# EmilyJrxx/YOLO_PPF_Pose_Estimation

Measured on AMD Instinct MI355X. Metric: PPF pair-matches/sec (accumulator votes) per cropped scene, higher is better.
Workload: dtype u32 votes / f64 pair features

## Files before the change

yolo_ppf_pose_estimation_amd/csrc/ppf_match_host.h:

```cpp
#ifndef PPF_MATCH_HOST_H
#define PPF_MATCH_HOST_H

extern "C" {

ppf_status ppf_workspace_create(ppf_workspace** out) {
  if (!out) return fail(PPF_ERR_INVALID, "ppf_workspace_create: NULL");
  *out = new (std::nothrow) ppf_workspace();
  if (!*out) return fail(PPF_ERR_NOMEM, "ppf_workspace_create: out of memory");
  return PPF_OK;
}
ppf_status ppf_workspace_destroy(ppf_workspace* ws) {
  if (!ws) return PPF_OK;
  delete ws;
  return PPF_OK;
}
ppf_status ppf_workspace_set_option(ppf_workspace* ws, int option, double value) {
  if (!ws) return fail(PPF_ERR_INVALID, "ppf_workspace_set_option: NULL");
  switch (option) {
    case PPF_OPT_HIT_FRACTION:
      if (!(value > 0 && value <= 1)) return fail(PPF_ERR_INVALID, "ppf_workspace_set_option: hit fraction must be in (0, 1]");
      ws->hit_frac = value;
      ws->frac_known = true;
      return PPF_OK;
    case PPF_OPT_GROUP_ROUND_BUCKETS:
      if (!(value >= 0 && value <= 1e9)) return fail(PPF_ERR_INVALID, "ppf_workspace_set_option: bad bucket count");
      ws->round_buckets_cap = (int)value;
      return PPF_OK;
    case PPF_OPT_CLUSTER_SERIAL:
      ws->cluster_serial = value != 0;
      return PPF_OK;
    case PPF_OPT_ACC32:
      if (!(value == 0 || value == 1 || value == 2 || value == 3)) return fail(PPF_ERR_INVALID, "ppf_workspace_set_option: PPF_OPT_ACC32 takes 0 .. 3");
      ws->force_acc32 = value == 1;
      ws->acc32_policy = value == 1 ? 0 : (int)value;
      ws->heavy_votes = ~0ull;
      if (value != 0) ws->acc32 = false;
      return PPF_OK;
    case PPF_OPT_BATCH_REFS:
      if (!(value >= 0 && value <= 1e9)) return fail(PPF_ERR_INVALID, "ppf_workspace_set_option: bad batch size");
      ws->batch_refs_cap = (int)value;
      return PPF_OK;
    case PPF_OPT_RUN_STAGING:
      if (!(value >= 0 && value <= 1e9)) return fail(PPF_ERR_INVALID, "ppf_workspace_set_option: bad run staging size");
      ws->run_seg_cap = (int)value;
      return PPF_OK;
    case PPF_OPT_TABLE_FRACTION:
      if (!(value > 0 && value <= 1)) return fail(PPF_ERR_INVALID, "ppf_workspace_set_option: table fraction must be in (0, 1]");
      ws->tbl_frac = std::min(TBL_FRAC_MAX, value);
      return PPF_OK;
    default:
      return fail(PPF_ERR_INVALID, "ppf_workspace_set_option: unknown option %d", option);
  }
}
ppf_status ppf_workspace_enable_timing(ppf_workspace* ws, int on) {
  if (!ws) return fail(PPF_ERR_INVALID, "ppf_workspace_enable_timing: NULL");
  if (on && !ws->ev[0])
    for (auto& e : ws->ev) HIPCHK(hipEventCreate(&e));
  ws->timing = on != 0;
  return PPF_OK;
}

static ppf_status check_match_args(const ppf_model* m, const void* scene, int ns, int sstride, int snoff, const void* edge, int ne,
                                   int estride, int enoff, const ppf_match_params* p) {
  if (!m) return fail(PPF_ERR_NOT_TRAINED, "The model is not trained. Cannot match without training");
  if (!scene || ns <= 0 || bad_layout(sstride, snoff) || !p) return fail(PPF_ERR_INVALID, "match: bad scene argument");
  if (edge && (ne <= 0 || bad_layout(estride, enoff))) return fail(PPF_ERR_INVALID, "match: bad edge argument");
  if (!(p->relative_scene_sample_step <= 1 && p->relative_scene_sample_step > 0))
    return fail(PPF_ERR_INVALID, "match: relativeSceneSampleStep must be in (0, 1]");
  if (!p->presampled && !(p->relative_scene_distance > 0)) return fail(PPF_ERR_INVALID, "match: relativeSceneDistance must be > 0");
  if (p->ref_stride < 1 || p->ref_offset < 0) return fail(PPF_ERR_INVALID, "match: bad ref_offset/ref_stride");
  int dev = 0;
  HIPCHK(hipGetDevice(&dev));
  if (dev != m->device)
    return fail(PPF_ERR_INVALID, "match: the model lives on device %d, the calling thread's current device is %d", m->device, dev);
  return PPF_OK;
}

static ppf_status prepare_scene(ppf_workspace* ws, const float* d_scene, int ns, int sstride, int snoff, const float* d_edge, int ne,
                                int estride, int enoff, const ppf_match_params* params, hipStream_t st) {
  auto load = [&](CloudDev& dst, const float* d_src, int rows, int stride, int noff) -> ppf_status {
    if (params->presampled) return dst.load_device(d_src, rows, stride, noff, st);
    return device_sample_cloud(d_src, rows, stride, noff, (float)params->relative_scene_distance, dst, nullptr, st);
  };
  ppf_status s = load(ws->surf, d_scene, ns, sstride, snoff);
  if (s != PPF_OK) return s;
  if (d_edge) s = load(ws->edge, d_edge, ne, estride, enoff);
  ws->has_edge = d_edge != nullptr;
  return s;
}

static ppf_status match_prepared(const ppf_model* m, ppf_workspace* ws, const ppf_match_params* params, hipStream_t st, bool retry = false);

ppf_status ppf_match_device(const ppf_model* m, ppf_workspace* ws, const float* d_scene, int ns, int sstride, int snoff,
                            const float* d_edge, int ne, int estride, int enoff, const ppf_match_params* params, void* stream) {
  if (!ws) return fail(PPF_ERR_INVALID, "ppf_match_device: workspace is NULL");
  if (!m) return fail(PPF_ERR_NOT_TRAINED, "The model is not trained. Cannot match without training");
  if (!have_device()) return fail(PPF_ERR_HIP, "ppf_match_device: no HIP device (this engine has no CPU fallback)");
  ppf_status s = check_match_args(m, d_scene, ns, sstride, snoff, d_edge, ne, estride, enoff, params);
  if (s != PPF_OK) return s;
  hipStream_t st = (hipStream_t)stream;
  s = prepare_scene(ws, d_scene, ns, sstride, snoff, d_edge, ne, estride, enoff, params, st);
  if (s != PPF_OK) return s;
  return match_prepared(m, ws, params, st);
}

static ppf_workspace::Learned* workspace_learned(ppf_workspace* ws, const ppf_model* m, bool create) {
  for (auto& fm : ws->frac_by_model)
    if (fm.model_serial == m->serial) return &fm;
  if (!create) return nullptr;
  if (ws->frac_by_model.size() >= 16) ws->frac_by_model.erase(ws->frac_by_model.begin());
  ws->frac_by_model.push_back({m->serial, 0.25, 0.4, TBL_FRAC_START});
  return &ws->frac_by_model.back();
}

static void workspace_remember_frac(ppf_workspace* ws) {
  if (!ws->model || !ws->frac_known) return;
  ppf_workspace::Learned* fm = workspace_learned(ws, ws->model, true);
  fm->hit = ws->hit_frac; fm->run = ws->run_frac; fm->tbl = ws->tbl_frac;
}

static void workspace_hold_model(ppf_workspace* ws, const ppf_model* m) {
  if (ws->model == m) return;
  ppf_model* old = ws->model;
  ws->model = const_cast<ppf_model*>(m);
  if (ws->model_owns_me) return;
  if (ws->model) ws->model->refcount.fetch_add(1);
  if (old) (void)ppf_model_release(old);
}

ppf_workspace::~ppf_workspace() {
  sync_device(device);
  for (auto& e : ev)
    if (e) (void)hipEventDestroy(e);
  for (auto& e : batch_ev)
    if (e) (void)hipEventDestroy(e);
  if (model && !model_owns_me) (void)ppf_model_release(model);
  if (h_sum) (void)hipHostFree(h_sum);
}

constexpr double HIT_SCRATCH_BYTES = 8.0 + 8.0 + 2.0 + 16.0 / 6.0;

static void launch_pairs(const MatchArgs& va, bool darboux, hipStream_t st) {
  const dim3 grid(va.pair_chunks, va.n_ref), block(PAIR_BLOCK);
  const dim3 ogrid((unsigned)std::min(va.n_ref, 1024)), oblock(256);
  if (darboux) {
    if (va.same_cloud) k_pairs<true, false><<<grid, block, 0, st>>>(va);
    else k_pairs<true, true><<<grid, block, 0, st>>>(va);
    if (!va.count_only) { if (va.same_cloud) k_pairs_odd<true, false><<<ogrid, oblock, 0, st>>>(va); else k_pairs_odd<true, true><<<ogrid, oblock, 0, st>>>(va); }
  } else {
    if (va.same_cloud) k_pairs<false, false><<<grid, block, 0, st>>>(va);
    else k_pairs<false, true><<<grid, block, 0, st>>>(va);
    if (!va.count_only) { if (va.same_cloud) k_pairs_odd<false, false><<<ogrid, oblock, 0, st>>>(va); else k_pairs_odd<false, true><<<ogrid, oblock, 0, st>>>(va); }
  }
}

static ppf_status match_prepared(const ppf_model* m, ppf_workspace* ws, const ppf_match_params* params, hipStream_t st, bool retry) {
  ppf_status s = PPF_OK;
  const bool d_edge = ws->has_edge;
  if (ws->model != m) {
    workspace_remember_frac(ws);
    ws->acc32 = false;
    ws->heavy_votes = ~0ull;
    if (const ppf_workspace::Learned* fm = workspace_learned(ws, m, false)) {
      ws->hit_frac = fm->hit; ws->run_frac = fm->run; ws->tbl_frac = fm->tbl;
      ws->frac_known = true;
    } else if (!ws->frac_by_model.empty()) {
      ws->frac_known = false;
    }
  }
  workspace_hold_model(ws, m);
  HIPCHK(hipGetDevice(&ws->device));
  ws->params = *params;
  ws->stream = st;
  ws->clustered = false;
  ws->checked = false;
  ws->sum_valid = false;
  ws->final_poses.clear();
  const int retries = retry ? ws->stats.n_retries : 0;
  memset(&ws->stats, 0, sizeof(ws->stats));
  ws->stats.n_retries = retries;
  const int rows = ws->surf.n;
  const int scene_step = (int)(1.0 / params->relative_scene_sample_step);
  const int n_ref_total = (rows + scene_step - 1) / scene_step;
  const int n_ref = n_ref_total > params->ref_offset ? (n_ref_total - params->ref_offset + params->ref_stride - 1) / params->ref_stride : 0;
  ws->rows = rows;
  ws->n_ref_total = n_ref_total;
  ws->n_ref = n_ref;
  ws->n_batches = 0;
  ws->stats.n_scene_sampled = rows;
  ws->stats.n_paired = d_edge ? ws->edge.n : rows;
  ws->stats.n_ref = n_ref;
  ws->pending = true;
  if (n_ref == 0) return PPF_OK;

  const int T = m->info.n_tiles;
  HIPCHK(ws->partial.reserve((size_t)n_ref * T * 2));
  HIPCHK(ws->half_edge.reserve((size_t)n_ref * T * 2));
  HIPCHK(ws->ovf_items.reserve((size_t)n_ref * T));
  if (ws->acc32_policy == 3) {
    HIPCHK(ws->item_votes.reserve((size_t)n_ref * T));
    HIPCHK(ws->need_hist.reserve(2 * ACC_HIST));
  }
  const size_t n_cnt = (size_t)n_ref * T + n_ref + 16;
  HIPCHK(ws->counters.reserve(n_cnt));
  HIPCHK(ws->votes.reserve(n_ref));
  HIPCHK(ws->raw_poses.reserve(n_ref));
  if (ws->timing) HIPCHK(hipEventRecord(ws->ev[0], st));
  if (ws->acc_dump)
    HIPCHK(hipMemsetAsync(ws->acc_dump, 0, (size_t)n_ref * (size_t)m->info.n_ref * (size_t)m->info.num_angles * sizeof(uint32_t), st));
  if (ws->acc32_policy == 3) {
    HIPCHK(hipMemsetAsync(ws->need_hist.p, 0, 2 * ACC_HIST * sizeof(unsigned long long), st));
    HIPCHK(hipMemsetAsync(ws->item_votes.p, 0, (size_t)n_ref * T * sizeof(unsigned long long), st));
  }

  MatchArgs va;
  memset(&va, 0, sizeof(va));
  va.surf = ws->surf.view();
  va.paired = d_edge ? ws->edge.view() : ws->surf.view();
  va.same_cloud = d_edge ? 0 : 1;
  va.scene_step = scene_step; va.ref_offset = params->ref_offset; va.ref_stride = params->ref_stride;
  va.slotmap = m->slotmap.p; va.slot_mask = m->info.slots - 1;
  va.key_lut = m->key_lut.p; va.kd = m->kd;
  va.bucket_off = m->bucket_off.p; va.n_buckets = (int)m->info.n_buckets;
  va.records = m->records.p;
  va.n_tiles = T; va.tile_refs = m->info.tile_refs; va.num_angles = m->info.num_angles; va.n_model = m->info.n_ref;
  va.angle_step = m->info.angle_step; va.dist_step = m->info.distance_step;
  va.partial = ws->partial.p;
  va.edge = ws->half_edge.p;
  va.ovf_items = ws->ovf_items.p;
  va.cellsum = ws->counters.p;
  va.pairs = ws->counters.p + (size_t)n_ref * T;
  va.tally = ws->counters.p + (size_t)n_ref * T + n_ref + 2;
  va.acc_dump = ws->acc_dump;
  va.bucket_total = m->bucket_total.p;
  va.bucket_mid = m->bucket_mid.p;
  va.key_exact = m->params.key_equality == PPF_KEY_EXACT;
  const bool acc32_all = ws->force_acc32 || (ws->acc32 && ws->acc32_policy == 0);
  va.item_votes = (!acc32_all && ws->acc32_policy == 3) ? ws->item_votes.p : nullptr;
  va.heavy_votes = ws->heavy_votes;
  const bool darboux = m->params.feature == PPF_FEATURE_DARBOUX;
  va.pair_radius = params->pair_radius;
  va.agg_min_hits = (params->vote_mode == PPF_VOTE_DIRECT || params->alpha_range_2pi || m->info.num_angles > AGG_MAX_ANGLES) ? 0 : PPF_AGG_MIN_HITS;
  const int n_paired = va.paired.n;
  va.pair_chunks = (n_paired + PAIR_BLOCK * PAIRS_PER_THREAD - 1) / (PAIR_BLOCK * PAIRS_PER_THREAD);
  const uint32_t round_cap = ws->round_buckets_cap > 0 ? (uint32_t)std::min(ws->round_buckets_cap, GROUP_MAX_BUCKETS) : (uint32_t)GROUP_MAX_BUCKETS;
  va.n_rounds = std::max(1, (int)((m->info.n_buckets + round_cap - 1) / round_cap));
  va.round_buckets = (int)std::min<uint32_t>(std::max<uint32_t>(m->info.n_buckets, 1u), round_cap);

  const bool cursors_new = !ws->cursors.p;
  HIPCHK(ws->cursors.reserve(CUR_WORDS));
  va.cursors = ws->cursors.p;
  if (cursors_new) HIPCHK(hipMemsetAsync(ws->cursors.p, 0, CUR_WORDS * sizeof(uint32_t), st));
  va.n_counters = n_cnt;
  va.n_ovf_items = (unsigned long long)n_ref * T;
  if (!ws->frac_known) {
    HIPCHK(hipMemsetAsync(ws->cursors.p, 0, CUR_WORDS * sizeof(uint32_t), st));
    va.count_only = 1;
    va.stripe_bits = 6;
    for (int base = 0; base < n_ref; base += 32768) {
      va.ref_base = base;
      va.n_ref = std::min(32768, n_ref - base);
      launch_pairs(va, darboux, st);
      HIPCHK(hipGetLastError());
    }
    va.count_only = 0;
    std::vector<uint32_t> cw(CUR_SORTED);
    HIPCHK(hipMemcpyAsync(cw.data(), ws->cursors.p, cw.size() * sizeof(uint32_t), hipMemcpyDeviceToHost, st));
    HIPCHK(host_stream_sync(st));
    unsigned long long hits = 0;
    for (int sidx = 0; sidx < POOL_STRIPES; sidx++)
      hits += (unsigned long long)cw[sidx * CUR_STRIDE] | ((unsigned long long)cw[sidx * CUR_STRIDE + 1] << 32);
    const double pairs_total = (double)n_ref * (double)n_paired;
    ws->hit_frac = std::min(1.0, std::max(1e-3, 1.06 * (double)hits / std::max(1.0, pairs_total)));
    ws->frac_known = true;
  }
  const double frac = std::min(1.0, std::max(ws->hit_frac, 1e-3));
  const double hits_per_ref = std::max(64.0, frac * (double)n_paired);
  const double tbl_frac = !va.agg_min_hits ? 0.0 : frac >= 1.0 ? TBL_FRAC_MAX : std::min(TBL_FRAC_MAX, ws->tbl_frac);
  int batch = (int)std::min<double>((double)n_ref, std::max(1.0, (double)HIT_BYTES_BUDGET / (hits_per_ref * (HIT_SCRATCH_BYTES + tbl_frac * TBL_BYTES))));
  batch = (int)std::min<double>((double)batch, std::max(1.0, 2.0e9 / hits_per_ref));
  batch = std::min(batch, 32768);
  if (ws->batch_refs_cap > 0) batch = std::min(batch, ws->batch_refs_cap);
  const bool worst_case = frac >= 1.0;
  const double est = hits_per_ref * (double)batch;
  const uint32_t wg_hits = PAIR_BLOCK * PAIRS_PER_THREAD;
  int stripe_bits = 6;
  while (stripe_bits > 0 && ((size_t)batch * va.pair_chunks >> stripe_bits) < 512) stripe_bits--;
  if (worst_case) stripe_bits = 0;
  const uint32_t n_stripes = 1u << stripe_bits;
  const uint32_t stripe_cap = worst_case ? (uint32_t)std::min<double>(4.0e9 / n_stripes, (double)batch * va.pair_chunks * wg_hits)
                                         : (uint32_t)(est / n_stripes * 1.04) + 2 * wg_hits;
  const uint32_t sorted_cap = (uint32_t)std::min(4.0e9, est + 4096.0);
  const uint32_t run_cap = worst_case ? sorted_cap : (uint32_t)std::min<double>((double)sorted_cap, std::max(est * std::min(1.0, ws->run_frac), 64.0 * batch) + 1024.0);
  HIPCHK(ws->frames.reserve((size_t)batch * 12));
  HIPCHK(ws->raw.fit((size_t)stripe_cap * n_stripes));
  HIPCHK(ws->chunk_desc.reserve((size_t)batch * va.pair_chunks));
  HIPCHK(ws->hit_count.reserve(batch));
  HIPCHK(ws->s_a64.fit(sorted_cap));
  const uint32_t table_cap = !va.agg_min_hits ? 1u : (uint32_t)std::min(1.0e9, std::max(est * (worst_case ? TBL_FRAC_MAX : tbl_frac), 4.0 * batch) + 256.0);
  HIPCHK(ws->runs.fit(run_cap));
  HIPCHK(ws->tables.fit((size_t)table_cap * TBL_BYTES));
  HIPCHK(ws->table_desc.fit(table_cap));
  HIPCHK(ws->run_blocks.reserve((size_t)batch * va.n_rounds));
  HIPCHK(ws->work.reserve(batch));
  HIPCHK(ws->perm.reserve(batch));
  HIPCHK(ws->perm_group.reserve(batch));
  HIPCHK(ws->ovf_list.reserve((size_t)batch * T));
  va.ovf_list = ws->ovf_list.p;
  ws->stats.scratch_bytes = ws->frames.bytes() + ws->raw.bytes() + ws->cursors.bytes() + ws->chunk_desc.bytes() + ws->hit_count.bytes() +
                            ws->s_a64.bytes() + ws->runs.bytes() + ws->run_blocks.bytes() + ws->tables.bytes() + ws->table_desc.bytes() +
                            ws->work.bytes() + ws->perm.bytes() + ws->perm_group.bytes();
  va.frames = ws->frames.p;
  va.raw = ws->raw.p; va.stripe_cap = stripe_cap; va.stripe_bits = stripe_bits;
  va.chunk_desc = ws->chunk_desc.p; va.hit_count = ws->hit_count.p;
  va.s_a64 = ws->s_a64.p; va.sorted_cap = sorted_cap;
  va.runs = ws->runs.p; va.run_cap = run_cap; va.run_blocks = ws->run_blocks.p;
  va.tables = ws->tables.p; va.table_desc = ws->table_desc.p; va.table_cap = table_cap;
  va.work = ws->work.p; va.perm = ws->perm.p; va.perm_group = ws->perm_group.p;

  const size_t acc_words = (size_t)vote_lds_words(m->info.tile_refs, m->info.num_angles);
  va.run_seg = vote_run_seg(acc_words, (size_t)LDS_BYTES);
  if (ws->run_seg_cap > 0) va.run_seg = std::max(64, std::min(va.run_seg, ws->run_seg_cap / 64 * 64));
  const size_t lds = vote_lds_fixed(va.run_seg) + acc_words * 4;
  if (lds > (size_t)LDS_BYTES) return fail(PPF_ERR_INVALID, "match: model tile of %d reference points does not fit the LDS accumulator", m->info.tile_refs);
  const size_t group_lds = (size_t)((va.round_buckets + 1) & ~1) * sizeof(uint32_t) + (size_t)((va.pair_chunks + 2) & ~1) * sizeof(uint32_t) * 2;
  if (group_lds + 2048 > (size_t)LDS_BYTES) return fail(PPF_ERR_INVALID, "match: %d paired points are more than one call can group", n_paired);
  static std::once_flag once;
  static hipError_t attr_err = hipSuccess;
  std::call_once(once, [] {
    const void* votes[4] = {reinterpret_cast<const void*>(&k_vote<false, false>), reinterpret_cast<const void*>(&k_vote<true, false>),
                            reinterpret_cast<const void*>(&k_vote<false, true>), reinterpret_cast<const void*>(&k_vote<true, true>)};
    for (const void* f : votes)
      if (attr_err == hipSuccess) attr_err = hipFuncSetAttribute(f, hipFuncAttributeMaxDynamicSharedMemorySize, LDS_BYTES);
    if (attr_err == hipSuccess)
      attr_err = hipFuncSetAttribute(reinterpret_cast<const void*>(&k_group), hipFuncAttributeMaxDynamicSharedMemorySize, LDS_BYTES - 1024);
  });
  HIPCHK(attr_err);
  const int n_batches = (n_ref + batch - 1) / batch;
  ws->n_batches = n_batches;
  ws->stats.n_batches = n_batches;
  if (ws->timing)
    while (ws->batch_ev.size() < ws->ev_base + (size_t)n_batches * 4) {
      hipEvent_t e = nullptr;
      HIPCHK(hipEventCreate(&e));
      ws->batch_ev.push_back(e);
    }
  for (int bi = 0; bi < n_batches; bi++) {
    const int base = bi * batch;
    va.ref_base = base;
    va.n_ref = std::min(batch, n_ref - base);
    va.first_batch = bi == 0;
    if (++ws->odd_epoch == 0u) {
      HIPCHK(hipMemsetAsync(ws->cursors.p + CUR_ODDVALUES, 0, sizeof(uint32_t), st));
      ws->odd_epoch = 1u;
    }
    va.odd_epoch = ws->odd_epoch;
#if PPF_ABL_GROUP != 1
    HIPCHK(hipMemsetAsync(ws->s_a64.p, 0, ws->s_a64.bytes(), st));
#endif
    k_frames<<<dim3(std::max((va.n_ref + 63) / 64, std::min((va.paired.n + 63) / 64, 1024))), dim3(64), 0, st>>>(va);
    HIPCHK(hipGetLastError());
    if (ws->timing) HIPCHK(hipEventRecord(ws->batch_ev[ws->ev_base + bi * 4 + 0], st));
    launch_pairs(va, darboux, st);
    HIPCHK(hipGetLastError());
    if (ws->timing) HIPCHK(hipEventRecord(ws->batch_ev[ws->ev_base + bi * 4 + 1], st));
    k_rank<<<dim3((va.n_ref + RANK_KEYS - 1) / RANK_KEYS), dim3(256), 0, st>>>(va.hit_count, va.n_ref, nullptr, ws->perm_group.p, nullptr);
    k_group<<<dim3(va.n_ref), dim3(GROUP_BLOCK), group_lds, st>>>(va);
    HIPCHK(hipGetLastError());
    if (va.agg_min_hits) {
      k_tables<<<dim3((table_cap + TABLE_BLOCK / 64 - 1) / (TABLE_BLOCK / 64)), dim3(TABLE_BLOCK), 0, st>>>(va);
      HIPCHK(hipGetLastError());
    }
    k_rank<<<dim3((va.n_ref + RANK_KEYS - 1) / RANK_KEYS), dim3(256), 0, st>>>(va.work, va.n_ref, nullptr, va.perm, nullptr);
    HIPCHK(hipGetLastError());
    if (ws->timing) HIPCHK(hipEventRecord(ws->batch_ev[ws->ev_base + bi * 4 + 2], st));
    const dim3 grid16((unsigned)((size_t)va.n_ref * T)), grid32((unsigned)((size_t)va.n_ref * T * 2));
    if (!acc32_all) {
      va.acc32 = 0;
      if (params->alpha_range_2pi) k_vote<true, false><<<grid16, dim3(VOTE_BLOCK), lds, st>>>(va);
      else k_vote<false, false><<<grid16, dim3(VOTE_BLOCK), lds, st>>>(va);
      HIPCHK(hipGetLastError());
    }
    va.acc32 = acc32_all ? 1 : 2;
    const dim3 g32 = acc32_all ? grid32 : dim3(std::min(grid32.x, 256u));
    if (params->alpha_range_2pi) k_vote<true, true><<<g32, dim3(VOTE_BLOCK), lds, st>>>(va);
    else k_vote<false, true><<<g32, dim3(VOTE_BLOCK), lds, st>>>(va);
    va.acc32 = 0;
    HIPCHK(hipGetLastError());
    if (ws->timing) HIPCHK(hipEventRecord(ws->batch_ev[ws->ev_base + bi * 4 + 3], st));
  }

  FinalArgs fa;
  fa.surf = ws->surf.view(); fa.model = m->cloud.view();
  fa.scene_step = scene_step; fa.ref_offset = params->ref_offset; fa.ref_stride = params->ref_stride; fa.n_ref = n_ref;
  fa.n_tiles = T; fa.tile_refs = m->info.tile_refs; fa.num_angles = m->info.num_angles;
  fa.alpha_2pi = params->alpha_range_2pi != 0;
  fa.acc32 = acc32_all ? 1 : 0; fa.ovf_items = ws->ovf_items.p; fa.edge = ws->half_edge.p;
// ... 474 lines not shown
```

yolo_ppf_pose_estimation_amd/csrc/ppf_match_kernels.h:

```cpp
#ifndef PPF_MATCH_KERNELS_H
#define PPF_MATCH_KERNELS_H

#ifndef PPF_GUARD_REL
#define PPF_GUARD_REL 5e-7f
#endif
#ifndef PPF_AGG_MIN_HITS
#define PPF_AGG_MIN_HITS 24
#endif
#ifndef PPF_AGG_MIN_RECORDS
#define PPF_AGG_MIN_RECORDS 32
#endif
#ifndef PPF_ABL_COUNTED
#define PPF_ABL_COUNTED 1
#endif
#ifndef PPF_ABL_OWNCELL
#define PPF_ABL_OWNCELL 1
#endif
#ifndef PPF_ABL_DIRECT_SMALL
#define PPF_ABL_DIRECT_SMALL 1
#endif
#ifndef PPF_ABL_DIRECT_BIG
#define PPF_ABL_DIRECT_BIG 1
#endif
#ifndef PPF_MOCK_PAIRBINS
// ... 39 lines not shown
#ifndef PPF_TWO_QUEUES
#define PPF_TWO_QUEUES 0
#endif
#ifndef PPF_PIPE_VALU
#define PPF_PIPE_VALU 4
#endif

constexpr int PAIR_BLOCK = 256;
#ifndef PPF_PAIRS_PER_THREAD
#define PPF_PAIRS_PER_THREAD 12
#endif
constexpr int PAIRS_PER_THREAD = PPF_PAIRS_PER_THREAD;
constexpr int VOTE_BLOCK = 1024;
constexpr int VOTE_WAVES = VOTE_BLOCK / 64;
constexpr int VOTE_UNROLL = 4;
constexpr int VOTE_CHUNK = 64 * VOTE_UNROLL * 4;
constexpr int VOTE_MAX_HITS = PPF_AGG_MIN_HITS;
#ifndef PPF_AGG_CHUNK
#define PPF_AGG_CHUNK 1024
#endif
constexpr int AGG_CHUNK = PPF_AGG_CHUNK;
constexpr int AGG_NY = 16;
constexpr int AGG_SUB = 191;
constexpr int AGG_MAX_ANGLES = 31;
#ifndef PPF_RUN_SEG
#define PPF_RUN_SEG 704
#endif
constexpr int RUN_SEG = PPF_RUN_SEG;
constexpr int RUN_SEG_MAX = 1024;
static_assert(RUN_SEG % 64 == 0 && RUN_SEG <= RUN_SEG_MAX && RUN_SEG_MAX == 1024, "the staging loop gives one thread to a run and scans whole waves");
constexpr int GROUP_BLOCK = 512;
#ifndef PPF_GROUP_MLP
#define PPF_GROUP_MLP 4
#endif
constexpr int GROUP_MLP = PPF_GROUP_MLP;
constexpr int GROUP_MAX_BUCKETS = 36000;
constexpr int POOL_STRIPES = 64;
constexpr int LDS_HEADER = 256;

constexpr int CUR_STRIDE = 32;
constexpr int CUR_SORTED = POOL_STRIPES * CUR_STRIDE;
constexpr int CUR_RUNS = CUR_SORTED + CUR_STRIDE;
constexpr int CUR_ODDVALUES = CUR_RUNS + CUR_STRIDE;
constexpr int CUR_OVFCOUNT = CUR_ODDVALUES + CUR_STRIDE;
constexpr int CUR_TABLES = CUR_OVFCOUNT + CUR_STRIDE;
constexpr int CUR_OVERFLOW = CUR_TABLES + CUR_STRIDE;
constexpr int CUR_WORDS = CUR_OVERFLOW + CUR_STRIDE;

constexpr int AGG_ROW = 20;
constexpr int AGG_ROW_CE = 17;
constexpr int AGG_SCRATCH = ((AGG_Q + 1) * AGG_ROW + 15) / 16 * 16;
constexpr int AGG_OFF_COLS = (AGG_Q + 1) * AGG_ROW;
constexpr uint32_t AGG_COLS_ALL = (2u << AGG_NY) - 1u;
static_assert(AGG_OFF_COLS % 4 == 0 && AGG_OFF_COLS + 4 <= AGG_SCRATCH, "the column mask lives in the padding behind the rows");
constexpr int TBL_OFF_A32 = AGG_SCRATCH;
constexpr int TBL_A32_BYTES = (AGG_NY * AGG_Q > 768 ? AGG_NY * AGG_Q : 768);
constexpr int TBL_OFF_IDX = TBL_OFF_A32 + TBL_A32_BYTES;
constexpr int TBL_BYTES = TBL_OFF_IDX + 192;
constexpr int AGG_OFF_CE = TBL_BYTES;
constexpr int TBL_BUILD_BYTES = AGG_OFF_CE + ((AGG_Q + 1) * 4 + 15) / 16 * 16;
static_assert(AGG_SUB * 4 <= 768 && AGG_SUB <= 192 && AGG_SUB < 256, "table hit range too long");
static_assert(AGG_SCRATCH % 16 == 0 && TBL_BYTES % 16 == 0, "tables are copied 16 bytes at a time");
constexpr int TABLE_BLOCK = 256;
constexpr double TBL_FRAC_MAX = 1.0 / PPF_AGG_MIN_HITS + 1.0 / AGG_SUB;
constexpr double TBL_FRAC_START = 0.02;

__device__ __forceinline__ float acos32_estimate(double x) {
  const double ax = ppf_fabs(x);
  const float xf = (float)ax;
  const float t = fmaxf((float)(1.0 - ax), 0.0f);
  float p = -0.001441536471247673f;
  p = __builtin_fmaf(p, xf, 0.007245631422847509f);
  p = __builtin_fmaf(p, xf, -0.01780921407043934f);
  p = __builtin_fmaf(p, xf, 0.03133561089634895f);
  p = __builtin_fmaf(p, xf, -0.0503128282725811f);
  p = __builtin_fmaf(p, xf, 0.08899927139282227f);
  p = __builtin_fmaf(p, xf, -0.21459989249706268f);
  p = __builtin_fmaf(p, xf, 1.5707963705062866f);
  const float a = __builtin_amdgcn_sqrtf(t) * p;
  return x >= 0.0 ? a : 3.14159274101257324f - a;
}

struct FastKeyConsts {
  float rstep32;
  float gq;
  double rdstep;
};

__device__ __forceinline__ void pair_key(const ppf_vec3& p1, const ppf_vec3& n1, const ppf_vec3& p2, const ppf_vec3& n2,
                                         const double angle_step, const double dist_step, const FastKeyConsts& fk, int32_t (&k)[4]) {
  const double dx = p2.x - p1.x, dy = p2.y - p1.y, dz = p2.z - p1.z;
  const double d2 = __builtin_fma(dz, dz, __builtin_fma(dy, dy, dx * dx));
  const double hd = 0.5 * d2;
  double rinv = __builtin_amdgcn_rsq(d2);
  rinv = rinv * __builtin_fma(-(hd * rinv), rinv, 1.5);
  rinv = rinv * __builtin_fma(-(hd * rinv), rinv, 1.5);
  const double f3 = d2 * rinv;
  const double x0 = __builtin_fma(n1.z, dz, __builtin_fma(n1.y, dy, n1.x * dx)) * rinv;
  const double x1 = __builtin_fma(n2.z, dz, __builtin_fma(n2.y, dy, n2.x * dx)) * rinv;
  const double x2 = __builtin_fma(n1.z, n2.z, __builtin_fma(n1.y, n2.y, n1.x * n2.x));
  bool slow = !(f3 > 2.0 * PPF_EPS) || !(ppf_fabs(x0) <= 1.0 - 1e-12) || !(ppf_fabs(x1) <= 1.0 - 1e-12) || !(ppf_fabs(x2) <= 1.0);
  {
    const float q0 = acos32_estimate(x0) * fk.rstep32, q1 = acos32_estimate(x1) * fk.rstep32,
                q2 = acos32_estimate(x2) * fk.rstep32;
    k[0] = (int)q0; k[1] = (int)q1; k[2] = (int)q2;
    const float lim = 0.5f - fk.gq;
    slow |= (__builtin_fabsf(__builtin_amdgcn_fractf(q0) - 0.5f) > lim) |
            (__builtin_fabsf(__builtin_amdgcn_fractf(q1) - 0.5f) > lim) |
            (__builtin_fabsf(__builtin_amdgcn_fractf(q2) - 0.5f) > lim);
    const double q3 = f3 * fk.rdstep;
    k[3] = (int)q3;
    const double fr3 = q3 - (double)k[3];
    slow |= !(fr3 > 1e-9 && fr3 < 1.0 - 1e-9) || !(q3 < 1.0e5);
  }
  if (slow) {
    double f[4] = {0, 0, 0, 0};
    ppf_pair_feature(p1, n1, p2, n2, f);
    k[0] = ppf_d2i(f[0] / angle_step); k[1] = ppf_d2i(f[1] / angle_step); k[2] = ppf_d2i(f[2] / angle_step);
    k[3] = ppf_d2i(f[3] / dist_step);
  }
}

__device__ __forceinline__ bool pair_key_darboux(const ppf_vec3& p1, const ppf_vec3& n1, const ppf_vec3& p2, const ppf_vec3& n2,
                                                 const double angle_step, const double dist_step, int32_t (&k)[4]) {
  double f[4];
  if (!ppf_pair_feature_darboux(p1, n1, p2, n2, f)) return false;
  k[0] = ppf_floor_key(f[0] / angle_step); k[1] = ppf_floor_key(f[1] / angle_step); k[2] = ppf_floor_key(f[2] / angle_step);
  k[3] = ppf_floor_key(f[3] / dist_step);
  return true;
}

struct MatchArgs {
  CloudSoA surf;
  CloudSoA paired;
  int same_cloud;
  int scene_step, ref_offset, ref_stride;
  int ref_base, n_ref;
  const SlotWord* slotmap;
  uint32_t slot_mask;
  const int32_t* key_lut;
  KeyDims kd;
  const uint32_t* bucket_off;
  int n_buckets;
  const uint4* records;
  int n_tiles, tile_refs, num_angles, n_model;
  double angle_step, dist_step;
  double* frames;
  uint2* raw;
  uint32_t stripe_cap;
  int stripe_bits;
  uint32_t* cursors;
  uint2* chunk_desc;
  int pair_chunks;
  unsigned long long* hit_count;
  double* s_a64;
  uint32_t sorted_cap;
  uint4* runs;
  unsigned char* tables;
  uint2* table_desc;
  uint32_t table_cap;
  uint32_t run_cap;
  uint2* run_blocks;
  int n_rounds, round_buckets;
  const uint32_t* bucket_total;
  const uint32_t* bucket_mid;
  unsigned long long* work;
  uint32_t* perm;
  const uint32_t* perm_group;
  int agg_min_hits;
  int key_exact;
  double pair_radius;
  int run_seg;
  int acc32;
  uint32_t* ovf_items;
  unsigned long long* item_votes;
  unsigned long long heavy_votes;
  uint32_t* ovf_list;
  int count_only;
  uint2* partial;
  uint32_t* edge;
  unsigned long long* cellsum;
  unsigned long long* pairs;
  unsigned long long* tally;
  uint32_t* acc_dump;
  uint32_t odd_epoch;
  int first_batch;
  unsigned long long n_counters;
  unsigned long long n_ovf_items;
};

__device__ __forceinline__ int ref_row(const MatchArgs& a, int r_local) {
  return (a.ref_offset + (a.ref_base + r_local) * a.ref_stride) * a.scene_step;
}

__global__ __launch_bounds__(64) void k_frames(MatchArgs a) {
  const int r = blockIdx.x * blockDim.x + threadIdx.x;
  bool odd = false;
  for (int j = r; j < a.paired.n; j += gridDim.x * blockDim.x) {
    const float m = (fabsf(a.paired.x[j]) + fabsf(a.paired.y[j])) + fabsf(a.paired.z[j]);
    odd |= !(m < 1e30f);
  }
  if (r < a.n_ref) {
    const int i = ref_row(a, r);
    double R[9], t[3];
    ppf_transform_rt(ld3(a.surf.x, a.surf.y, a.surf.z, i), ld3(a.surf.nx, a.surf.ny, a.surf.nz, i), R, t);
    double* f = a.frames + (size_t)r * 12;
#pragma unroll
    for (int k = 0; k < 9; k++) { f[k] = R[k]; odd |= !(ppf_fabs(R[k]) < 1e30); }
#pragma unroll
    for (int k = 0; k < 3; k++) { f[9 + k] = t[k]; odd |= !(ppf_fabs(t[k]) < 1e30); }
  }
  if (odd) atomicExch(&a.cursors[CUR_ODDVALUES], a.odd_epoch);
  const size_t g0 = (size_t)r, gs = (size_t)gridDim.x * blockDim.x;
  for (size_t k = g0; k < (size_t)(a.first_batch ? CUR_WORDS : CUR_OVERFLOW); k += gs)
    if (k != (size_t)CUR_ODDVALUES) a.cursors[k] = 0u;
  if (a.agg_min_hits)
    for (size_t k = g0; k < (size_t)a.table_cap; k += gs) a.table_desc[k] = make_uint2(0u, 0u);
  if (a.first_batch) {
    for (size_t k = g0; k < (size_t)a.n_counters; k += gs) a.cellsum[k] = 0ull;
    for (size_t k = g0; k < (size_t)a.n_ovf_items; k += gs) a.ovf_items[k] = 0u;
  }
}

__device__ __forceinline__ uint32_t pool_stripe(const uint32_t wg, const int stripe_bits) {
  return stripe_bits ? (wg * 2654435761u) >> (32 - stripe_bits) : 0u;
}

template <bool DARBOUX, bool S2B>
__global__ __launch_bounds__(PAIR_BLOCK) void k_pairs(MatchArgs a) {
  __shared__ uint2 stash[PAIRS_PER_THREAD][PAIR_BLOCK];
  __shared__ uint32_t wtot[PAIR_BLOCK / 64];
  __shared__ uint32_t wg_base;
  const int r = blockIdx.y;
  const int tid = threadIdx.x, lane = tid & 63, wave = tid >> 6;
  const int i_ref = ref_row(a, r);
  const ppf_vec3 p1 = ld3(a.surf.x, a.surf.y, a.surf.z, i_ref), n1 = ld3(a.surf.nx, a.surf.ny, a.surf.nz, i_ref);
  FastKeyConsts fk;
  fk.rstep32 = (float)(1.0 / a.angle_step);
  fk.gq = 4.0e-6f * fk.rstep32;
  fk.rdstep = 1.0 / a.dist_step;
  unsigned long long my_pairs = 0;
  uint32_t hit_mask = 0;
  const int j0 = blockIdx.x * (PAIR_BLOCK * PAIRS_PER_THREAD) + tid;
  const int n = a.paired.n;
  float nx0 = 0, nx1 = 0, nx2 = 0, nx3 = 0, nx4 = 0, nx5 = 0;
  auto ldf = [](const float* __restrict__ base, const uint32_t byte_off) { return *reinterpret_cast<const float*>(reinterpret_cast<const char*>(base) + byte_off); };
  {
    const uint32_t jc = (uint32_t)min(j0, n - 1) * 4u;
    nx0 = ldf(a.paired.x, jc); nx1 = ldf(a.paired.y, jc); nx2 = ldf(a.paired.z, jc);
    nx3 = ldf(a.paired.nx, jc); nx4 = ldf(a.paired.ny, jc); nx5 = ldf(a.paired.nz, jc);
  }
#pragma unroll 2
  for (int it = 0; it < PAIRS_PER_THREAD; it++) {
    const int j = j0 + it * PAIR_BLOCK;
    const ppf_vec3 p2 = ppf_mk3((double)nx0, (double)nx1, (double)nx2), n2 = ppf_mk3((double)nx3, (double)nx4, (double)nx5);
    {
      const uint32_t jn = (uint32_t)min(j + PAIR_BLOCK, n - 1) * 4u;
      nx0 = ldf(a.paired.x, jn); nx1 = ldf(a.paired.y, jn); nx2 = ldf(a.paired.z, jn);
      nx3 = ldf(a.paired.nx, jn); nx4 = ldf(a.paired.ny, jn); nx5 = ldf(a.paired.nz, jn);
    }
    if (j < n && (S2B || j != i_ref)) {
      const bool self_pair = S2B && p2.x == p1.x && p2.y == p1.y && p2.z == p1.z && n2.x == n1.x && n2.y == n1.y && n2.z == n1.z;
      bool skip = self_pair;
      if (__builtin_expect(a.pair_radius > 0.0, 0)) {
        const double dx = p2.x - p1.x, dy = p2.y - p1.y, dz = p2.z - p1.z;
        skip |= ppf_sqrt(dx * dx + dy * dy + dz * dz) > a.pair_radius;
      }
      if (!skip) {
        int32_t key[4];
        bool valid = true;
        if (DARBOUX) valid = pair_key_darboux(p1, n1, p2, n2, a.angle_step, a.dist_step, key);
        else pair_key(p1, n1, p2, n2, a.angle_step, a.dist_step, fk, key);
        if (valid) {
          int b;
          size_t ki;
          if (key_index(a.kd, key[0], key[1], key[2], key[3], &ki)) {
            b = a.key_lut[ki];
          } else if (a.key_exact) {
            b = key_index_nan(a.kd, key[0], key[1], key[2], key[3], &ki) ? a.key_lut[ki] : -1;
          } else {
            b = slot_to_bucket(a.slotmap, ppf_murmur_key16(key[0], key[1], key[2], key[3]) & a.slot_mask);
          }
          my_pairs += 1u;
          if (b >= 0) {
            stash[it][tid] = make_uint2((uint32_t)b, (uint32_t)j);
            hit_mask |= 1u << it;
          }
        }
      }
    }
  }
  const uint32_t mine = (uint32_t)__popc(hit_mask);
  uint32_t incl = mine;
#pragma unroll
  for (int o = 1; o < 64; o <<= 1) {
    const uint32_t y = __shfl_up(incl, o);
    if (lane >= o) incl += y;
  }
  if (lane == 63) wtot[wave] = incl;
  __syncthreads();
  uint32_t woff = 0, total = 0;
#pragma unroll
  for (int k = 0; k < PAIR_BLOCK / 64; k++) {
    const uint32_t w = wtot[k];
    if (k < wave) woff += w;
    total += w;
  }
  if (a.count_only) {
    if (tid == 0 && total) {
      const uint32_t stripe = pool_stripe(blockIdx.y * gridDim.x + blockIdx.x, a.stripe_bits);
      atomicAdd(reinterpret_cast<unsigned long long*>(&a.cursors[stripe * CUR_STRIDE]), (unsigned long long)total);
    }
    return;
  }
  if (tid == 0) {
    uint32_t base = 0xFFFFFFFFu;
    if (total) {
      const uint32_t stripe = pool_stripe(blockIdx.y * gridDim.x + blockIdx.x, a.stripe_bits);
      const uint32_t b = atomicAdd(&a.cursors[stripe * CUR_STRIDE], total);
      if (b <= a.stripe_cap && total <= a.stripe_cap - b) base = stripe * a.stripe_cap + b;
      else atomicOr(&a.cursors[CUR_OVERFLOW], 1u);
    }
    wg_base = base;
    a.chunk_desc[(size_t)r * a.pair_chunks + blockIdx.x] = base == 0xFFFFFFFFu ? make_uint2(0u, 0u) : make_uint2(base, total);
  }
  __syncthreads();
  const uint32_t base = wg_base;
  if (base != 0xFFFFFFFFu) {
    uint32_t pos = base + woff + incl - mine;
#pragma unroll 1
    for (int it = 0; it < PAIRS_PER_THREAD; it++) {
      if (hit_mask & (1u << it)) a.raw[pos++] = stash[it][tid];
    }
  }
#pragma unroll
  for (int o = 32; o > 0; o >>= 1) my_pairs += __shfl_down(my_pairs, o);
  if (lane == 0 && my_pairs) atomicAdd(&a.pairs[a.ref_base + r], my_pairs);
}

template <bool DARBOUX, bool S2B>
__global__ __launch_bounds__(256) void k_pairs_odd(MatchArgs a) {
  for (int r = blockIdx.x * 4 + (threadIdx.x >> 6); r < a.n_ref; r += gridDim.x * 4) {
    unsigned long long s = 0;
    for (int c = threadIdx.x & 63; c < a.pair_chunks; c += 64) s += a.chunk_desc[(size_t)r * a.pair_chunks + c].y;
#pragma unroll
    for (int o = 32; o > 0; o >>= 1) s += __shfl_down(s, o);
    if ((threadIdx.x & 63) == 0) a.hit_count[r] = s;
  }
  if (a.cursors[CUR_ODDVALUES] != a.odd_epoch) return;
  const int lane = threadIdx.x & 63;
  for (int r = blockIdx.x; r < a.n_ref; r += gridDim.x) {
    const int i_ref = ref_row(a, r);
    const ppf_vec3 p1 = ld3(a.surf.x, a.surf.y, a.surf.z, i_ref), n1 = ld3(a.surf.nx, a.surf.ny, a.surf.nz, i_ref);
    const double* f = a.frames + (size_t)r * 12;
    unsigned long long gone = 0;
    for (int j = threadIdx.x; j < a.paired.n; j += blockDim.x) {
      if (!(S2B || j != i_ref)) continue;
      const ppf_vec3 p2 = ld3(a.paired.x, a.paired.y, a.paired.z, j), n2 = ld3(a.paired.nx, a.paired.ny, a.paired.nz, j);
      const bool self_pair = S2B && p2.x == p1.x && p2.y == p1.y && p2.z == p1.z && n2.x == n1.x && n2.y == n1.y && n2.z == n1.z;
      bool skip = self_pair;
      if (a.pair_radius > 0.0) {
        const double dx = p2.x - p1.x, dy = p2.y - p1.y, dz = p2.z - p1.z;
        skip |= ppf_sqrt(dx * dx + dy * dy + dz * dz) > a.pair_radius;
      }
      if (skip) continue;
      if (DARBOUX) {
        int32_t key[4];
        if (!pair_key_darboux(p1, n1, p2, n2, a.angle_step, a.dist_step, key)) continue;
      }
      const double qy = f[10] + (f[3] * p2.x + f[4] * p2.y + f[5] * p2.z);
      const double qz = f[11] + (f[6] * p2.x + f[7] * p2.y + f[8] * p2.z);
      if (!ppf_alpha_exists(qy, qz)) gone += 1ull;
    }
#pragma unroll
    for (int o = 32; o > 0; o >>= 1) gone += __shfl_down(gone, o);
    if (lane == 0 && gone) atomicAdd(&a.pairs[a.ref_base + r], 0ull - gone);
  }
}

__device__ __forceinline__ uint32_t hit_cell(const double alpha_s, const double s64) {
  const double y = alpha_s * s64;
  const double Y = __builtin_floor(y);
  int p = (int)((y - Y) * (double)AGG_Q);
  p = min(max(p, 0), AGG_Q - 1);
  const int yy = min(max((int)Y + 8, 0), AGG_NY - 1);
  return (uint32_t)(yy * AGG_Q + p);
}

__global__ __launch_bounds__(GROUP_BLOCK) void k_group(MatchArgs a) {
  extern __shared__ __align__(8) uint32_t gcnt[];
  __shared__ unsigned long long wsum[GROUP_BLOCK / 64];
  __shared__ uint32_t wtot[4][GROUP_BLOCK / 64];
  __shared__ uint32_t sh[5];
  const int r = a.perm_group ? (int)a.perm_group[blockIdx.x] : (int)blockIdx.x;
  const int tid = threadIdx.x, lane = tid & 63, wave = tid >> 6;
  uint32_t* cpre = gcnt + ((a.round_buckets + 1) & ~1);
  uint32_t* cbase = cpre + ((a.pair_chunks + 2) & ~1);
  const uint32_t n_raw = (uint32_t)a.hit_count[r];
  const uint2* __restrict__ desc = a.chunk_desc + (size_t)r * a.pair_chunks;
  if (tid == 0) {
    uint32_t base = 0, ok = 1;
    if (n_raw) {
      base = atomicAdd(&a.cursors[CUR_SORTED], n_raw);
      if (!(base <= a.sorted_cap && n_raw <= a.sorted_cap - base)) { ok = 0; atomicOr(&a.cursors[CUR_OVERFLOW], 2u); }
    }
    sh[0] = base; sh[1] = ok;
  }
  if (wave == 1) {
    uint32_t run = 0;
    for (int c0 = 0; c0 < a.pair_chunks; c0 += 64) {
      const int c = c0 + lane;
      const uint32_t v = c < a.pair_chunks ? desc[c].y : 0u;
      uint32_t incl = v;
#pragma unroll
      for (int o = 1; o < 64; o <<= 1) {
        const uint32_t y = __shfl_up(incl, o);
        if (lane >= o) incl += y;
      }
      if (c < a.pair_chunks) { cpre[c] = run + incl - v; cbase[c] = desc[c].x; }
      run += __shfl(incl, 63);
    }
    if (lane == 0) cpre[a.pair_chunks] = run;
  }
  __syncthreads();
  const uint32_t hit_base = sh[0];
  const bool ok = sh[1] != 0;
  const double* __restrict__ fr = a.frames + (size_t)r * 12;
  const double R10 = fr[3], R11 = fr[4], R12 = fr[5], R20 = fr[6], R21 = fr[7], R22 = fr[8], ty = fr[10], tz = fr[11];
  const uint32_t agg_min = a.agg_min_hits > 0 ? (uint32_t)a.agg_min_hits : 0xFFFFFFFFu;
  const uint32_t n_list = ok ? n_raw : 0u;
  const bool check_alpha = a.cursors[CUR_ODDVALUES] == a.odd_epoch;
  unsigned long long w = 0;
  uint32_t placed = 0, runs_written = 0, tables_given = 0;
  for (int round = 0; round < a.n_rounds; round++) {
    const uint32_t b0 = (uint32_t)round * (uint32_t)a.round_buckets;
    const uint32_t nb = min((uint32_t)a.round_buckets, (uint32_t)a.n_buckets - b0);
    for (uint32_t k = tid; k < nb; k += GROUP_BLOCK) gcnt[k] = 0;
    __syncthreads();
    {
      int c = 0;
      for (uint32_t g0 = tid; g0 < n_list; g0 += GROUP_MLP * GROUP_BLOCK) {
        uint32_t at[GROUP_MLP];
        uint2 key[GROUP_MLP];
#pragma unroll
        for (int u = 0; u < GROUP_MLP; u++) {
          const uint32_t g = g0 + (uint32_t)u * GROUP_BLOCK;
          const uint32_t gc = min(g, n_list - 1u);
          while (gc >= cpre[c + 1]) c++;
          at[u] = cbase[c] + (gc - cpre[c]);
          key[u] = a.raw[at[u]];
          if (g >= n_list) key[u].x = 0xFFFFFFFFu;
        }
        ppf_vec3 p2[GROUP_MLP];
        bool in[GROUP_MLP];
#pragma unroll
        for (int u = 0; u < GROUP_MLP; u++) {
          in[u] = key[u].x - b0 < nb;
          p2[u] = ppf_mk3(0.0, 0.0, 0.0);
          if (in[u] && check_alpha) p2[u] = ld3(a.paired.x, a.paired.y, a.paired.z, (int)key[u].y);
        }
#pragma unroll
        for (int u = 0; u < GROUP_MLP; u++) {
          if (in[u]) {
            bool has_alpha = true;
            if (check_alpha) {
              const double qy = ty + (R10 * p2[u].x + R11 * p2[u].y + R12 * p2[u].z);
              const double qz = tz + (R20 * p2[u].x + R21 * p2[u].y + R22 * p2[u].z);
              has_alpha = ppf_alpha_exists(qy, qz);
            }
            if (has_alpha) {
              atomicAdd(&gcnt[key[u].x - b0], 1u);
            } else {
              a.raw[at[u]].x = 0xFFFFFFFFu;
            }
          }
        }
      }
    }
    __syncthreads();
    const uint32_t per = (nb + GROUP_BLOCK - 1) / GROUP_BLOCK;
    const uint32_t k0 = min((uint32_t)tid * per, nb), k1 = min(k0 + per, nb);
    uint32_t th = 0, tH = 0, tL = 0, tT = 0;
    for (uint32_t k = k0; k < k1; k++) {
      const uint32_t c = gcnt[k];
      th += c;
      if (c) { if (c >= agg_min) { tH++; tT += (c + AGG_SUB - 1) / AGG_SUB; } else tL++; }
    }
    uint32_t ih = th, iH = tH, iL = tL, iT = tT;
#pragma unroll
    for (int o = 1; o < 64; o <<= 1) {
// ... 1165 lines not shown
```

Measured before the change: 13780 billion.

## Make pair workgroups span several chunks and overlap cursor atomics with compute

Each k_pairs workgroup now walks up to four consecutive pair chunks instead of one, keeping stash entries in a shared-memory ring. A chunk's global cursor atomic and raw writes are deferred and flushed partway through the next chunk, so atomic latency is hidden behind key computation. The stash now holds only the 32-bit bucket (the index j is rebuilt at flush time), the key constants are precomputed on the host, and launch bounds request higher occupancy. In exchange the grid is smaller, so parallelism drops for small scenes, control flow and barriers become more complex, and stripe selection now hashes per chunk rather than per block.

```diff
diff --git a/yolo_ppf_pose_estimation_amd/csrc/ppf_match_host.h b/yolo_ppf_pose_estimation_amd/csrc/ppf_match_host.h
--- a/yolo_ppf_pose_estimation_amd/csrc/ppf_match_host.h
+++ b/yolo_ppf_pose_estimation_amd/csrc/ppf_match_host.h
@@ -141,7 +141,7 @@
 constexpr double HIT_SCRATCH_BYTES = 8.0 + 8.0 + 2.0 + 16.0 / 6.0;
 
 static void launch_pairs(const MatchArgs& va, bool darboux, hipStream_t st) {
-  const dim3 grid(va.pair_chunks, va.n_ref), block(PAIR_BLOCK);
+  const dim3 grid((va.pair_chunks + va.span_chunks - 1) / va.span_chunks, va.n_ref), block(PAIR_BLOCK);
   const dim3 ogrid((unsigned)std::min(va.n_ref, 1024)), oblock(256);
   if (darboux) {
     if (va.same_cloud) k_pairs<true, false><<<grid, block, 0, st>>>(va);
@@ -243,6 +243,10 @@
   va.agg_min_hits = (params->vote_mode == PPF_VOTE_DIRECT || params->alpha_range_2pi || m->info.num_angles > AGG_MAX_ANGLES) ? 0 : PPF_AGG_MIN_HITS;
   const int n_paired = va.paired.n;
   va.pair_chunks = (n_paired + PAIR_BLOCK * PAIRS_PER_THREAD - 1) / (PAIR_BLOCK * PAIRS_PER_THREAD);
+  va.span_chunks = pair_span_chunks(va.pair_chunks);
+  va.fk_rstep32 = (float)(1.0 / va.angle_step);
+  va.fk_gq = 4.0e-6f * va.fk_rstep32;
+  va.fk_rdstep = 1.0 / va.dist_step;
   const uint32_t round_cap = ws->round_buckets_cap > 0 ? (uint32_t)std::min(ws->round_buckets_cap, GROUP_MAX_BUCKETS) : (uint32_t)GROUP_MAX_BUCKETS;
   va.n_rounds = std::max(1, (int)((m->info.n_buckets + round_cap - 1) / round_cap));
   va.round_buckets = (int)std::min<uint32_t>(std::max<uint32_t>(m->info.n_buckets, 1u), round_cap);
diff --git a/yolo_ppf_pose_estimation_amd/csrc/ppf_match_kernels.h b/yolo_ppf_pose_estimation_amd/csrc/ppf_match_kernels.h
--- a/yolo_ppf_pose_estimation_amd/csrc/ppf_match_kernels.h
+++ b/yolo_ppf_pose_estimation_amd/csrc/ppf_match_kernels.h
@@ -215,6 +215,9 @@
   uint32_t* cursors;
   uint2* chunk_desc;
   int pair_chunks;
+  int span_chunks;
+  float fk_rstep32, fk_gq;
+  double fk_rdstep;
   unsigned long long* hit_count;
   double* s_a64;
   uint32_t sorted_cap;
@@ -289,9 +292,21 @@
   return stripe_bits ? (wg * 2654435761u) >> (32 - stripe_bits) : 0u;
 }
 
+constexpr int PAIR_SPAN_CHUNKS = 4;
+__host__ __device__ inline int pair_span_chunks(const int pair_chunks) {
+  const int quarter = (pair_chunks + 3) / 4;
+  return quarter < PAIR_SPAN_CHUNKS ? quarter : PAIR_SPAN_CHUNKS;
+}
+
+constexpr int PAIR_RING = 16;
+constexpr int PAIR_FLUSH_AT = PAIR_RING - PAIRS_PER_THREAD - 1;
+static_assert(PAIRS_PER_THREAD < PAIR_RING && (PAIR_RING & (PAIR_RING - 1)) == 0, "the ring needs a spare slot");
+static_assert(PAIR_BLOCK * PAIRS_PER_THREAD < 65536 && PAIRS_PER_THREAD <= 16, "a thread's offset in its sub-chunk and its hit mask share a word");
+
 template <bool DARBOUX, bool S2B>
-__global__ __launch_bounds__(PAIR_BLOCK) void k_pairs(MatchArgs a) {
-  __shared__ uint2 stash[PAIRS_PER_THREAD][PAIR_BLOCK];
+__global__ __launch_bounds__(PAIR_BLOCK, DARBOUX ? 4 : 5) void k_pairs(MatchArgs a) {
+  __shared__ uint32_t stash[PAIR_RING][PAIR_BLOCK];
+  __shared__ uint32_t carried[PAIR_BLOCK];
   __shared__ uint32_t wtot[PAIR_BLOCK / 64];
   __shared__ uint32_t wg_base;
   const int r = blockIdx.y;
@@ -299,106 +314,129 @@
   const int i_ref = ref_row(a, r);
   const ppf_vec3 p1 = ld3(a.surf.x, a.surf.y, a.surf.z, i_ref), n1 = ld3(a.surf.nx, a.surf.ny, a.surf.nz, i_ref);
   FastKeyConsts fk;
-  fk.rstep32 = (float)(1.0 / a.angle_step);
-  fk.gq = 4.0e-6f * fk.rstep32;
-  fk.rdstep = 1.0 / a.dist_step;
-  unsigned long long my_pairs = 0;
-  uint32_t hit_mask = 0;
-  const int j0 = blockIdx.x * (PAIR_BLOCK * PAIRS_PER_THREAD) + tid;
+  fk.rstep32 = a.fk_rstep32; fk.gq = a.fk_gq; fk.rdstep = a.fk_rdstep;
+  uint32_t my_pairs = 0;
   const int n = a.paired.n;
+  const int c0 = blockIdx.x * a.span_chunks, c1 = min(c0 + a.span_chunks, a.pair_chunks);
+  const int rows_all = (n + PAIR_BLOCK - 1) / PAIR_BLOCK;
+  int j = c0 * (PAIR_BLOCK * PAIRS_PER_THREAD) + tid;
   float nx0 = 0, nx1 = 0, nx2 = 0, nx3 = 0, nx4 = 0, nx5 = 0;
   auto ldf = [](const float* __restrict__ base, const uint32_t byte_off) { return *reinterpret_cast<const float*>(reinterpret_cast<const char*>(base) + byte_off); };
   {
-    const uint32_t jc = (uint32_t)min(j0, n - 1) * 4u;
+    const uint32_t jc = (uint32_t)min(j, n - 1) * 4u;
     nx0 = ldf(a.paired.x, jc); nx1 = ldf(a.paired.y, jc); nx2 = ldf(a.paired.z, jc);
     nx3 = ldf(a.paired.nx, jc); nx4 = ldf(a.paired.ny, jc); nx5 = ldf(a.paired.nz, jc);
   }
-#pragma unroll 2
-  for (int it = 0; it < PAIRS_PER_THREAD; it++) {
-    const int j = j0 + it * PAIR_BLOCK;
-    const ppf_vec3 p2 = ppf_mk3((double)nx0, (double)nx1, (double)nx2), n2 = ppf_mk3((double)nx3, (double)nx4, (double)nx5);
-    {
-      const uint32_t jn = (uint32_t)min(j + PAIR_BLOCK, n - 1) * 4u;
-      nx0 = ldf(a.paired.x, jn); nx1 = ldf(a.paired.y, jn); nx2 = ldf(a.paired.z, jn);
-      nx3 = ldf(a.paired.nx, jn); nx4 = ldf(a.paired.ny, jn); nx5 = ldf(a.paired.nz, jn);
-    }
-    if (j < n && (S2B || j != i_ref)) {
-      const bool self_pair = S2B && p2.x == p1.x && p2.y == p1.y && p2.z == p1.z && n2.x == n1.x && n2.y == n1.y && n2.z == n1.z;
-      bool skip = self_pair;
-      if (__builtin_expect(a.pair_radius > 0.0, 0)) {
-        const double dx = p2.x - p1.x, dy = p2.y - p1.y, dz = p2.z - p1.z;
-        skip |= ppf_sqrt(dx * dx + dy * dy + dz * dz) > a.pair_radius;
-      }
-      if (!skip) {
-        int32_t key[4];
-        bool valid = true;
-        if (DARBOUX) valid = pair_key_darboux(p1, n1, p2, n2, a.angle_step, a.dist_step, key);
-        else pair_key(p1, n1, p2, n2, a.angle_step, a.dist_step, fk, key);
-        if (valid) {
-          int b;
-          size_t ki;
-          if (key_index(a.kd, key[0], key[1], key[2], key[3], &ki)) {
-            b = a.key_lut[ki];
-          } else if (a.key_exact) {
-            b = key_index_nan(a.kd, key[0], key[1], key[2], key[3], &ki) ? a.key_lut[ki] : -1;
-          } else {
-            b = slot_to_bucket(a.slotmap, ppf_murmur_key16(key[0], key[1], key[2], key[3]) & a.slot_mask);
-          }
-          my_pairs += 1u;
-          if (b >= 0) {
-            stash[it][tid] = make_uint2((uint32_t)b, (uint32_t)j);
-            hit_mask |= 1u << it;
+  uint32_t slot = 0;
+  uint32_t pend = 0, prev_total = 0;
+  bool have_prev = false;
+  auto flush = [&](const int cp) {
+    if (tid == 0) {
+      uint32_t base = 0xFFFFFFFFu;
+      if (prev_total) {
+        const uint32_t stripe = pool_stripe((uint32_t)(r * a.pair_chunks + cp), a.stripe_bits);
+        if (pend <= a.stripe_cap && prev_total <= a.stripe_cap - pend) base = stripe * a.stripe_cap + pend;
+        else atomicOr(&a.cursors[CUR_OVERFLOW], 1u);
+      }
+      wg_base = base;
+      a.chunk_desc[(size_t)r * a.pair_chunks + cp] = base == 0xFFFFFFFFu ? make_uint2(0u, 0u) : make_uint2(base, prev_total);
+    }
+    __syncthreads();
+    const uint32_t base = wg_base;
+    if (base != 0xFFFFFFFFu) {
+      const uint32_t prev = carried[tid];
+      uint32_t pos = base + (prev & 0xFFFFu);
+      const uint32_t s0 = slot - PAIRS_PER_THREAD;
+      const uint32_t jp = (uint32_t)(cp * (PAIR_BLOCK * PAIRS_PER_THREAD) + tid);
+#pragma unroll 1
+      for (int it = 0; it < PAIRS_PER_THREAD; it++) {
+        if (prev & (0x10000u << it)) a.raw[pos++] = make_uint2(stash[(s0 + it) & (PAIR_RING - 1)][tid], jp + (uint32_t)(it * PAIR_BLOCK));
+      }
+    }
+    have_prev = false;
+  };
+#pragma unroll 1
+  for (int c = c0; c < c1; c++) {
+    const int rows = min(PAIRS_PER_THREAD, rows_all - c * PAIRS_PER_THREAD);
+    uint32_t hit_mask = 0;
+#pragma unroll 1
+    for (int it = 0; it < rows; it++, j += PAIR_BLOCK) {
+      const ppf_vec3 p2 = ppf_mk3((double)nx0, (double)nx1, (double)nx2), n2 = ppf_mk3((double)nx3, (double)nx4, (double)nx5);
+      {
+        const uint32_t jn = (uint32_t)min(j + PAIR_BLOCK, n - 1) * 4u;
+        nx0 = ldf(a.paired.x, jn); nx1 = ldf(a.paired.y, jn); nx2 = ldf(a.paired.z, jn);
+        nx3 = ldf(a.paired.nx, jn); nx4 = ldf(a.paired.ny, jn); nx5 = ldf(a.paired.nz, jn);
+      }
+      if (j < n && (S2B || j != i_ref)) {
+        const bool self_pair = S2B && p2.x == p1.x && p2.y == p1.y && p2.z == p1.z && n2.x == n1.x && n2.y == n1.y && n2.z == n1.z;
+        bool skip = self_pair;
+        if (__builtin_expect(a.pair_radius > 0.0, 0)) {
+          const double dx = p2.x - p1.x, dy = p2.y - p1.y, dz = p2.z - p1.z;
+          skip |= ppf_sqrt(dx * dx + dy * dy + dz * dz) > a.pair_radius;
+        }
+        if (!skip) {
+          int32_t key[4];
+          bool valid = true;
+          if (DARBOUX) valid = pair_key_darboux(p1, n1, p2, n2, a.angle_step, a.dist_step, key);
+          else pair_key(p1, n1, p2, n2, a.angle_step, a.dist_step, fk, key);
+          if (valid) {
+            int b;
+            size_t ki;
+            if (key_index(a.kd, key[0], key[1], key[2], key[3], &ki)) {
+              b = a.key_lut[ki];
+            } else if (a.key_exact) {
+              b = key_index_nan(a.kd, key[0], key[1], key[2], key[3], &ki) ? a.key_lut[ki] : -1;
+            } else {
+              b = slot_to_bucket(a.slotmap, ppf_murmur_key16(key[0], key[1], key[2], key[3]) & a.slot_mask);
+            }
+            my_pairs += 1u;
+            if (b >= 0) {
+              if (!a.count_only) stash[(slot + it) & (PAIR_RING - 1)][tid] = (uint32_t)b;
+              hit_mask |= 1u << it;
+            }
           }
         }
       }
-    }
-  }
-  const uint32_t mine = (uint32_t)__popc(hit_mask);
-  uint32_t incl = mine;
-#pragma unroll
-  for (int o = 1; o < 64; o <<= 1) {
-    const uint32_t y = __shfl_up(incl, o);
-    if (lane >= o) incl += y;
-  }
-  if (lane == 63) wtot[wave] = incl;
-  __syncthreads();
-  uint32_t woff = 0, total = 0;
-#pragma unroll
-  for (int k = 0; k < PAIR_BLOCK / 64; k++) {
-    const uint32_t w = wtot[k];
-    if (k < wave) woff += w;
-    total += w;
-  }
-  if (a.count_only) {
-    if (tid == 0 && total) {
-      const uint32_t stripe = pool_stripe(blockIdx.y * gridDim.x + blockIdx.x, a.stripe_bits);
-      atomicAdd(reinterpret_cast<unsigned long long*>(&a.cursors[stripe * CUR_STRIDE]), (unsigned long long)total);
-    }
-    return;
-  }
-  if (tid == 0) {
-    uint32_t base = 0xFFFFFFFFu;
-    if (total) {
-      const uint32_t stripe = pool_stripe(blockIdx.y * gridDim.x + blockIdx.x, a.stripe_bits);
-      const uint32_t b = atomicAdd(&a.cursors[stripe * CUR_STRIDE], total);
-      if (b <= a.stripe_cap && total <= a.stripe_cap - b) base = stripe * a.stripe_cap + b;
-      else atomicOr(&a.cursors[CUR_OVERFLOW], 1u);
-    }
-    wg_base = base;
-    a.chunk_desc[(size_t)r * a.pair_chunks + blockIdx.x] = base == 0xFFFFFFFFu ? make_uint2(0u, 0u) : make_uint2(base, total);
-  }
-  __syncthreads();
-  const uint32_t base = wg_base;
-  if (base != 0xFFFFFFFFu) {
-    uint32_t pos = base + woff + incl - mine;
-#pragma unroll 1
-    for (int it = 0; it < PAIRS_PER_THREAD; it++) {
-      if (hit_mask & (1u << it)) a.raw[pos++] = stash[it][tid];
-    }
-  }
-#pragma unroll
-  for (int o = 32; o > 0; o >>= 1) my_pairs += __shfl_down(my_pairs, o);
-  if (lane == 0 && my_pairs) atomicAdd(&a.pairs[a.ref_base + r], my_pairs);
+      if (it == PAIR_FLUSH_AT && have_prev) flush(c - 1);
+    }
+    if (have_prev) flush(c - 1);
+    const uint32_t mine = (uint32_t)__popc(hit_mask);
+    uint32_t incl = mine;
+#pragma unroll
+    for (int o = 1; o < 64; o <<= 1) {
+      const uint32_t y = __shfl_up(incl, o);
+      if (lane >= o) incl += y;
+    }
+    if (a.count_only) {
+      if (lane == 63 && incl) {
+        const uint32_t stripe = pool_stripe((uint32_t)(r * a.pair_chunks + c), a.stripe_bits);
+        atomicAdd(reinterpret_cast<unsigned long long*>(&a.cursors[stripe * CUR_STRIDE]), (unsigned long long)incl);
+      }
+      continue;
+    }
+    if (lane == 63) wtot[wave] = incl;
+    __syncthreads();
+    uint32_t woff = 0, total = 0;
+#pragma unroll
+    for (int k = 0; k < PAIR_BLOCK / 64; k++) {
+      const uint32_t w = wtot[k];
+      if (k < wave) woff += w;
+      total += w;
+    }
+    prev_total = __builtin_amdgcn_readfirstlane(total);
+    if (tid == 0 && prev_total) {
+      const uint32_t stripe = pool_stripe((uint32_t)(r * a.pair_chunks + c), a.stripe_bits);
+      pend = atomicAdd(&a.cursors[stripe * CUR_STRIDE], prev_total);
+    }
+    carried[tid] = (woff + incl - mine) | (hit_mask << 16);
+    slot += PAIRS_PER_THREAD;
+    have_prev = true;
+  }
+  if (have_prev) flush(c1 - 1);
+  unsigned long long wave_pairs = my_pairs;
+#pragma unroll
+  for (int o = 32; o > 0; o >>= 1) wave_pairs += __shfl_down(wave_pairs, o);
+  if (lane == 0 && wave_pairs) atomicAdd(&a.pairs[a.ref_base + r], wave_pairs);
 }
 
 template <bool DARBOUX, bool S2B>
```

Result: no change. 13740 billion (-0.3%).
